# Bojian-Wei/Non-IID-Distributed-Learning-with-Optimal-Mixture-Weights

Hardware: AMD Instinct MI355X
Metric: client-rounds/sec (whole node) (higher is better)
Workload: dtype f32; 1 GPU; config 2: fedavg, 100 clients x 512 rows, RFF D=2048, C=10, E=2, B=32, 10000 test rows, round=1880, parallel clients; algo=fedavg, clients_total=100, clients_per_gpu=100, rows_per_client=512, D=2048, C=10, epochs=2, batch=32, test_rows=10000, parallelism=clients1

## Files before the change

non-iid-distributed-learning-with-optimal-mixture-weights_amd/csrc/local_train_host.cpp:

```cpp
#include <mutex>
#include <unordered_map>

#include "local_train_wide.h"
#include "split_common.h"

namespace fs {

static_assert(SP_ERR_BYTES == PR_ERR_BYTES && SP_ERR_BYTES == PP_ERR_BYTES && SP_ERR_BYTES == WD_ERR_BYTES,
              "one error block for every form");

static int device_cus() {
  static int cus = 0;
  if (cus == 0) {
    int dev = 0;
    if (hipGetDevice(&dev) != hipSuccess) return 0;
    if (hipDeviceGetAttribute(&cus, hipDeviceAttributeMultiprocessorCount, dev) != hipSuccess) cus = 0;
  }
  return cus;
}

static unsigned exchange_generation(const void* ws, bool long_launch) {
  static std::mutex gm;
  static std::unordered_map<const void*, unsigned> gens;
  std::lock_guard<std::mutex> lk(gm);
  auto it = gens.find(ws);
  const unsigned prev = it == gens.end() ? 0u : it->second;
  const unsigned gen = (long_launch || prev >= 4095u) ? 0u : prev + 1u;
  gens[ws] = gen;
  return gen;
}

static unsigned spin_bound(unsigned form_limit) {
  const fs_tuning t = tuning();
  if (t.inject_timeout) return 0u;
  return t.spin_limit ? t.spin_limit : form_limit;
}

constexpr int SPLIT_PD_WIDE = 16, SPLIT_PD_NARROW = 0;
static int split_poll_delay(int G, bool chained) {
  const int t = tuning().split_poll_delay;
  if (t < 0) return 0;
  if (t > 0) return t;
  if (chained) return 0;
  return G >= 8 ? SPLIT_PD_WIDE : SPLIT_PD_NARROW;
}


static size_t split_dyn_lds(int RT, int NT, int G, int teams) {
  const int tiles = (NT + G - 1) / G;
  return sizeof(float) * (size_t)teams * (size_t)(RT * 16) * (size_t)(tiles * 64 + 8);
}

static size_t split_static_lds(int RT, int NW, int teams) {
  const int NR = RT * 16;
  return (size_t)teams * ((size_t)NW * NR * 16 * 4 + 2 * (size_t)NR * 16 * 4 + 2 * NR * 4 + NW * 3 * 4 + 8) + 64 +
         4 * teams;
}

static bool split_fits(int C, int B, int NT, int G, int teams) {
  if (!(G == 2 || G == 4 || G == 8 || G == 16)) return false;
  if (C > 16 || B > 32 || NT < G) return false;
  const int RT = lt_rt(B);
  const int nw = SP_WAVES / teams;
  const int tiles = (NT + G - 1) / G;
  if ((tiles + nw - 1) / nw > SP_TPW) return false;
  if (G >= 8 && RT * 16 * C + 2 > 512) return false;
  return split_dyn_lds(RT, NT, G, teams) + split_static_lds(RT, nw, teams) <= 160 * 1024;
}

static size_t pair_dyn_lds(int RT) { return sizeof(float) * 2 * (size_t)(RT * 16) * (size_t)(PR_TILES * 64 + 8); }

static size_t pair_static_lds(int RT) {
  const int NR = RT * 16;
  return (size_t)PR_WAVES * NR * 16 * 4 + (size_t)NR * 16 * 4 + 2 * NR * 4 + 2 * PR_WAVES * 2 * 4 +
         PR_WAVES * 4 + 8 + 64;
}

struct Form {
  int flag;
  int kernel;
  int lanes;
  int slots;
  bool chains;
  bool poll_delay;
  unsigned spin_limit;
  size_t fuse_lds;
  bool (*fits)(int C, int B, int NT, int G);
  int (*sz)(int RT);
  size_t (*lds)(int RT, int NT, int G);
  int (*launch)(const LTParams& P, int G, const SplitWS& X, int grid, size_t lds, hipStream_t st);
  const char* unfit;
};

static int split_sz(int RT) { return RT * 16 * 16 + 4; }
constexpr size_t SPLIT_FUSE_LDS = sizeof(float) * SP_WAVES * 16 * 17;

static const Form SPLIT = {
    0, FS_LT_SPLIT, 1, 2, true, true, SP_SPIN_LIMIT, SPLIT_FUSE_LDS,
    [](int C, int B, int NT, int G) { return split_fits(C, B, NT, G, 1); }, split_sz,
    [](int RT, int NT, int G) { return split_dyn_lds(RT, NT, G, 1); }, launch_split_instance,
    "fs_local_train: slice too wide for one workgroup"};

static const Form TEAMS = {
    FS_G_TEAMS, FS_LT_TEAMS, 2, 4, false, true, SP_SPIN_LIMIT, SPLIT_FUSE_LDS,
    [](int C, int B, int NT, int G) { return (G == 4 || G == 8) && split_fits(C, B, NT, G, 2); }, split_sz,
    [](int RT, int NT, int G) { return split_dyn_lds(RT, NT, G, 2); }, launch_teams_instance,
    "fs_local_train: slice too wide for one workgroup"};

static const Form PAIR = {
    FS_G_PAIR, FS_LT_PAIR, 2, 5, false, false, PR_SPIN_LIMIT, 0,
    [](int C, int B, int NT, int G) {
      if (!(G == 2 || G == 4 || G == 8 || G == 16)) return false;
      if (C > 14 || B > 32 || NT != PR_TILES * G) return false;
      const int RT = lt_rt(B);
      return pair_dyn_lds(RT) + pair_static_lds(RT) <= 160 * 1024;
    },
    [](int RT) { return RT * 16 * 16 + 4 >= PR_THREADS ? RT * 16 * 16 + 4 : PR_THREADS; },
    [](int RT, int, int) { return pair_dyn_lds(RT); }, launch_pair_instance,
    "fs_local_train: the pair form needs C <= 14, B <= 32 and ld == 512 G"};

static const Form PIPE = {
    FS_G_PIPE, FS_LT_PIPE, 1, 2, true, false, SP_SPIN_LIMIT, 0,
    [](int C, int B, int NT, int G) {
      if (!(G == 2 || G == 4 || G == 8 || G == 16)) return false;
      return C >= 1 && C <= 16 && B > 16 && B <= 32 && NT == PP_NTS * G;
    },
    [](int) { return PP_SZ; },
    [](int, int, int) { return sizeof(float) * (size_t)PP_NR * PP_RS; }, launch_pipe_instance,
    "fs_local_train: the pipe form needs ld = 1024 G (G = 2, 4, 8 or 16), 16 < B <= 32 and C <= 16"};

static const Form& form_of(int G) {
  return (G & FS_G_PIPE) ? PIPE : (G & FS_G_PAIR) ? PAIR : (G & FS_G_TEAMS) ? TEAMS : SPLIT;
}

static int form_groups(const Form& f, int N, int G, int chained, int cus) {
  return chained ? 1 : std::max(1, std::min((N + f.lanes - 1) / f.lanes, cus / G));
}

static int64_t form_xbuf_bytes(const Form& f, int ngroups, int G, int RT) {
  return (int64_t)ngroups * f.slots * G * f.sz(RT) * 8;
}

static int64_t form_ws_bytes(const Form& f, int N, int G, int B, int chained, int cus) {
  return form_xbuf_bytes(f, form_groups(f, N, G, chained, cus), G, lt_rt(B)) + SP_ERR_BYTES;
}

int split_idle_cus(int N, int C, int B, int64_t ld, int G, int chained) {
  if (G & FS_G_WIDE) return 0;
  const Form& f = form_of(G);
  const int g = G & (FS_G_PAIR - 1);
  const int cus = device_cus();
  if (chained || cus <= 0 || !f.fits(C, B, (int)(ld >> 6), g)) return 0;
  return std::max(0, cus - form_groups(f, N, g, 0, cus) * g);
}


static int form_admits(const Form& f, const LTParams& P, int G, int NT) {
  if (&f == &TEAMS && (P.chained || !(G == 4 || G == 8)))
    return fail(FS_EUNSUPPORTED, "fs_local_train: the team form runs parallel clients at G = 4 or 8");
  if (&f == &PAIR && P.chained) return fail(FS_EINVAL, "fs_local_train: the pair form needs parallel clients");
  if (&f == &SPLIT || &f == &TEAMS) {
    if (!(G == 2 || G == 4 || G == 8 || G == 16)) return fail(FS_EINVAL, "fs_local_train: G must be 1, 2, 4, 8 or 16");
    if (P.C > 16 || P.B > 32) return fail(FS_EUNSUPPORTED, "fs_local_train: split clients need C <= 16, B <= 32");
    if (NT < G) return fail(FS_EUNSUPPORTED, "fs_local_train: fewer feature tiles than workgroups per client");
  }
  if (!f.fits(P.C, P.B, NT, G)) return fail(FS_EUNSUPPORTED, f.unfit);
  return FS_OK;
}

static int exchange_setup(const Form& f, const LTParams& P, int G, void* ws, int64_t ws_bytes, hipStream_t st,
                          SplitWS& X, int& grid, size_t& lds) {
  const int RT = lt_rt(P.B);
  const int NT = (int)(P.ld >> 6);
  if (int rc = form_admits(f, P, G, NT)) return rc;
  const int cus = device_cus();
  if (cus <= 0) return fail(FS_EHIP, "fs_local_train: no device");
  if (G > cus) return fail(FS_EUNSUPPORTED, "fs_local_train: G exceeds the CU count");
  const int ng = form_groups(f, P.N, G, P.chained, cus);
  const int64_t xbytes = form_xbuf_bytes(f, ng, G, RT);
  if (!ws || ws_bytes < xbytes + SP_ERR_BYTES) return fail(FS_EINVAL, "fs_local_train: workspace too small");
  char* base = reinterpret_cast<char*>(ws);
  X.xbuf = reinterpret_cast<unsigned long long*>(base);
  X.err = reinterpret_cast<unsigned*>(base + ws_bytes - SP_ERR_BYTES);
  X.SZ = f.sz(RT);
  X.ngroups = ng;
  X.spin_limit = spin_bound(f.spin_limit);
  X.poll_delay = f.poll_delay ? split_poll_delay(G, P.chained != 0) : 0;
  X.stamps = nullptr;
#ifdef FS_STAMPS
  X.stamps = reinterpret_cast<unsigned long long*>(base + xbytes);
#endif
  const int64_t seq_clients = P.chained ? P.N : (P.N + ng * f.lanes - 1) / (ng * f.lanes);
  const bool long_launch = P.max_client_steps <= 0 || P.max_client_steps * seq_clients >= (1 << 20) - 1;
  const unsigned gen = exchange_generation(ws, long_launch);
  X.tag_base = gen << 20;
  if (gen <= 1) {
    hipError_t e = hipMemsetAsync(base, 0, (size_t)xbytes, st);
// ... 153 lines not shown
```

non-iid-distributed-learning-with-optimal-mixture-weights_amd/csrc/local_train_split.hip:

```cpp
#include <type_traits>

#include "common.h"
#include "eval_rows.h"
#include "lanes.h"
#include "split_common.h"

namespace fs {

#ifndef SP_E1
#define SP_E1 6
#endif
#ifndef SP_E2
#define SP_E2 0
#endif
#ifndef SP_E3
#define SP_E3 0
#endif
constexpr int SP_EARLY = SP_E1 + SP_E2 + SP_E3;
#ifndef SP_BWD_FENCE
#define SP_BWD_FENCE 1
#endif
#ifndef SP_BWD_NUM
#define SP_BWD_NUM 1
#endif
#ifndef SP_BWD_DEN
#define SP_BWD_DEN 1
#endif
#ifndef SP_BWD_PF
#define SP_BWD_PF 1
#endif
#ifndef SP_EG2
#define SP_EG2 4
#endif
#ifndef SP_BWD_TAIL
#define SP_BWD_TAIL 8
#endif
#ifndef SP_BWD_TAILPER
#define SP_BWD_TAILPER 8
#endif
#ifndef SP_MB_RSP
#define SP_MB_RSP 4
#endif
#ifndef SP_MB_BWD_PF
#define SP_MB_BWD_PF 1
#endif
#ifndef SP_MB_PRE
#define SP_MB_PRE 1
#endif

#ifdef FS_STAMPS
#define SP_STAMP(k)                                                                       \
  {                                                                                       \
    __builtin_amdgcn_sched_barrier(0);                                                    \
    unsigned long long t_;                                                                \
    asm volatile("s_memtime %0\n\ts_waitcnt lgkmcnt(0)" : "=s"(t_)::"memory");           \
    __builtin_amdgcn_sched_barrier(0);                                                    \
    if (k > 0) stamp_acc[k > 0 ? k - 1 : 0] += t_ - stamp_prev;                           \
    stamp_prev = t_;                                                                      \
  }
#else
#define SP_STAMP(k)
#endif

template <int CBSZ, int ABID, int BLGP>
__device__ __forceinline__ floatx4 mfma4x4(float a, float b, floatx4 c) {
  return __builtin_amdgcn_mfma_f32_4x4x1f32(a, b, c, CBSZ, ABID, BLGP);
}
template <int Q, int RT, int CB>
__device__ __forceinline__ void mb_fwd_q(floatx4 (&acc)[RT][CB], const float4 (&xt)[RT][4], const float4 (&wt)[CB]) {
#pragma unroll
  for (int e = 0; e < 4; ++e)
#pragma unroll
    for (int rt = 0; rt < RT; ++rt)
#pragma unroll
      for (int cb = 0; cb < CB; ++cb) acc[rt][cb] = mfma4x4<2, Q, 0>(comp(wt[cb], e), comp(xt[rt][Q], e), acc[rt][cb]);
}
template <int CB>
__device__ __forceinline__ void mb_bwd_row(floatx4 (&ga)[CB], float a, float g) {
  ga[0] = mfma4x4<0, 0, 4>(a, g, ga[0]);
  if constexpr (CB > 1) ga[1] = mfma4x4<0, 0, 5>(a, g, ga[1]);
  if constexpr (CB > 2) ga[2] = mfma4x4<0, 0, 6>(a, g, ga[2]);
  if constexpr (CB > 3) ga[3] = mfma4x4<0, 0, 7>(a, g, ga[3]);
}
__device__ __forceinline__ void mb_swap32(float& a, float& b) {
  const auto r = __builtin_amdgcn_permlane32_swap(__float_as_uint(a), __float_as_uint(b), false, false);
  a = __uint_as_float(r[0]);
  b = __uint_as_float(r[1]);
}
__device__ __forceinline__ void mb_swap16(float& a, float& b) {
  const auto r = __builtin_amdgcn_permlane16_swap(__float_as_uint(a), __float_as_uint(b), false, false);
  a = __uint_as_float(r[0]);
  b = __uint_as_float(r[1]);
}
__device__ __forceinline__ float mb_kgroup_sum(floatx4 a) {
  float r0 = a[0], r1 = a[1], r2 = a[2], r3 = a[3];
  mb_swap32(r0, r1);
  mb_swap32(r2, r3);
  float s01 = r0 + r1, s23 = r2 + r3;
  mb_swap16(s01, s23);
  return s01 + s23;
}
__device__ __forceinline__ int mb_perm(int lg) { return ((lg & 1) << 1) | (lg >> 1); }
template <int CB>
__device__ __forceinline__ int zp_off_mb(int r, int c) {
  return ((r >> 4) * CB + (c >> 2)) * 64 + (c & 3) * 16 + ((r & 15) ^ ((c >> 2) << 2));
}

template <int RT, int G, bool PROX, int EARLY, int TEAMS, int WAVES = SP_WAVES, int TPWK = SP_TPW, int MBK = 0>
__global__ __launch_bounds__(WAVES * 64, 1) void local_train_split_kernel(LTParams P, SplitWS X) {
  static_assert(TEAMS == 1 || TEAMS == 2, "teams");
  static_assert(WAVES == SP_WAVES || (WAVES == 4 && TEAMS == 1), "waves");
  static_assert(MBK >= 0 && MBK <= 4 && (MBK == 0 || TEAMS == 1), "mb");
  constexpr bool MB = MBK > 0;
  constexpr int NQ = MB ? MBK : 4;
  constexpr int NCS = !MB || MBK > 2 ? 16 : 4 * MBK;
  constexpr int NW = WAVES / TEAMS;
  constexpr int NTH = NW * 64;
  constexpr int NC = 16;
  constexpr int NR = RT * 16;
  constexpr int NZ = NR * NC;
  constexpr int NZS = NR * NCS;
  constexpr int TPW = TPWK;
  constexpr int XT = NTH;
  constexpr int M = ((G >= 8 ? 512 : NZ + 2) + XT - 1) / XT;
  constexpr int HC = G;
  __shared__ __attribute__((aligned(16))) float zpart_t[TEAMS][NW][NR * NC];
  __shared__ float gbuf_t[TEAMS][NR][NC];
  __shared__ float zsum_t[TEAMS][NR][NC];
  __shared__ int lab_t[TEAMS][2][NR];
  __shared__ float wred_t[TEAMS][NW][2];
  __shared__ float wce_t[TEAMS][NW];
  __shared__ float nrm_t[TEAMS][2];
  __shared__ unsigned tbar[TEAMS];
  extern __shared__ __attribute__((aligned(16))) float xs_dyn[];

  const int team = TEAMS > 1 ? __builtin_amdgcn_readfirstlane((int)threadIdx.x / NTH) : 0;
  const int tid = (int)threadIdx.x - team * NTH, lane = tid & 63, l16 = lane & 15, lg = lane >> 4;
  const int w = __builtin_amdgcn_readfirstlane(tid >> 6);
  const int mq = (lane >> 2) & 3, mi = lane & 3;
  auto& zpart = zpart_t[team];
  auto& gbuf = gbuf_t[team];
  auto& zsum = zsum_t[team];
  auto& lab = lab_t[team];
  auto& wred = wred_t[team];
  auto& wce = wce_t[team];
  auto& nrm = nrm_t[team];
  const int64_t ld = P.ld;
  const int NT = (int)(ld >> 6);
  const int C = P.C, B = P.B, E = P.E;
  const int NV = NR * C + 2;
  static_assert(NZS % 64 == 0, "the softmax loop must stay wave-uniform");

  const int nb = gridDim.x - P.fuse_E;
  if ((int)blockIdx.x >= nb) {
    if constexpr (WAVES == SP_WAVES)
      eval_persistent<SP_WAVES>(P.fuse_phi, P.ld, P.fuse_y, P.fuse_n, P.W_start, P.C, (int)blockIdx.x - nb, P.fuse_E,
                         xs_dyn, P.fuse_part);
    return;
  }
  int lin;
  if (P.chained) {
    if (blockIdx.x % 8) return;
    lin = blockIdx.x / 8;
  } else {
    lin = blockIdx.x;
    if (nb % 8 == 0) lin = (blockIdx.x % 8) * (nb / 8) + blockIdx.x / 8;
  }
  const int ngp = X.ngroups;
  const int grpp = lin / G, g = lin % G;
  if (grpp >= ngp) return;
  const int ng = ngp * TEAMS, grp = grpp * TEAMS + team;
  const int T = P.chained ? P.N : (P.N + ng - 1) / ng;
  const int t0 = tile_lo(g, G, NT), t1 = tile_lo(g + 1, G, NT);
  const int NTS = t1 - t0;
  constexpr int RSP = MB ? SP_MB_RSP : 8;
  const int RS = NTS * 64 + RSP;
  const int xs_off = TEAMS > 1 ? team * (NR * RS) : 0;
#define xs_lds (xs_dyn + xs_off)
  const float* start = P.W_start;
  unsigned long long* xb = X.xbuf + (int64_t)grp * 2 * G * X.SZ;
  unsigned tb_target = 0;
  bool tb_dead = false;
  if (TEAMS > 1 && tid == 0) tbar[team] = 0u;
  auto team_sync = [&]() {
    if constexpr (TEAMS == 1) {
      lds_barrier();
    } else {
      tb_target += NW;
      asm volatile("s_waitcnt lgkmcnt(0)" ::: "memory");
      if (lane == 0) __hip_atomic_fetch_add(&tbar[team], 1u, __ATOMIC_RELAXED, __HIP_MEMORY_SCOPE_WORKGROUP);
      for (unsigned sp = 0; !tb_dead &&
                            __hip_atomic_load(&tbar[team], __ATOMIC_RELAXED, __HIP_MEMORY_SCOPE_WORKGROUP) < tb_target;) {
        if (++sp > 64u * SP_SPIN_LIMIT) {
          if (lane == 0) __hip_atomic_store(X.err, 1u, __ATOMIC_RELAXED, __HIP_MEMORY_SCOPE_AGENT);
          tb_dead = true;
        }
        __builtin_amdgcn_s_sleep(1);
      }
      asm volatile("" ::: "memory");
    }
  };
  const float4 zero4 = make_float4(0.f, 0.f, 0.f, 0.f);

  float4 wr[TPW][NQ];
  const float* anc = P.W_start;
  auto wbase = [&]() {
    int64_t b = MB ? (int64_t)mi * ld + 64 * t0 + 16 * mq + 4 * lg : (int64_t)l16 * ld + 64 * t0 + 4 * lg;
    asm volatile("" : "+v"(b));
    return b;
  };
  auto woff = [&](int Tl, int q) -> int64_t { return MB ? 4 * q * ld + 64 * Tl : 64 * Tl + 16 * q; };
  auto wok = [&](int Tl, int q) { return Tl < NTS && (MB ? 4 * q + mi < C : l16 < C); };
  auto load_start = [&]() {
    const int64_t base = wbase();
    float s = 0.f;
#pragma unroll
    for (int i = 0; i < TPW; ++i) {
      const int Tl = w + NW * i;
#pragma unroll
      for (int q = 0; q < NQ; ++q) {
        wr[i][q] = wok(Tl, q) ? ld4(start + base + woff(Tl, q)) : zero4;
        s = sq4_acc(s, wr[i][q].x, wr[i][q].y, wr[i][q].z, wr[i][q].w);
      }
    }
    return wave_sum_dpp(s, lane);
  };
  auto store_w = [&](float* Wj) {
    const int64_t base = wbase();
#pragma unroll
    for (int i = 0; i < TPW; ++i) {
      const int Tl = w + NW * i;
#pragma unroll
      for (int q = 0; q < NQ; ++q)
        if (wok(Tl, q)) st4(Wj + base + woff(Tl, q), wr[i][q]);
    }
  };
  const float nw0 = load_start();
  if (lane == 0) { wred[w][0] = 0.f; wred[w][1] = nw0; }

  float4 xf[TPW][RT][4];
  int pn[RT], lb[RT];
  SpCur lc;
  bool lc_ok = sp_seek(lc, P, grp, ng, T, 0);
  auto fetch_raw = [&](int* raw, int64_t& base) {
    const int e_ = lc.st / lc.nbat, s_ = lc.st - e_ * lc.nbat;
    const int b0_ = s_ * B, bc_ = min(B, lc.n - b0_);
    const int32_t* pp_ = P.perms + (int64_t)E * lc.row0 + (int64_t)e_ * lc.n + b0_;
    base = lc.row0;
#pragma unroll
    for (int rt = 0; rt < RT; ++rt) {
      const int r_ = rt * 16 + l16;
      raw[rt] = pp_[r_ < bc_ ? r_ : 0];
    }
  };
  auto fetch_rows = [&]() {
    int raw[RT];
    int64_t base;
    fetch_raw(raw, base);
#pragma unroll
    for (int rt = 0; rt < RT; ++rt) pn[rt] = (int)(base + raw[rt]);
  };
#define SP_XLOAD()                                                                   \
  {                                                                                  \
    _Pragma("unroll") for (int rt = 0; rt < RT; ++rt) {                              \
      const int64_t r_ = pn[rt];                                                     \
      if (w == 0 && lg == 0) lb[rt] = P.labels[r_];                                  \
      const float* src_ = P.phi + r_ * ld + 64 * t0 + 4 * lg;                        \
      _Pragma("unroll") for (int i = 0; i < TPW; ++i)                                \
        if (w + NW * i < NTS)                                                        \
          _Pragma("unroll") for (int q = 0; q < 4; ++q)                              \
            xf[i][rt][q] = ld4(src_ + 64 * (w + NW * i) + 16 * q);                   \
    }                                                                                \
  }
  if (lc_ok) {
    fetch_rows();
    SP_XLOAD();
    lc_ok = sp_advance(lc, P, grp, ng, T);
    if (lc_ok) fetch_rows();
  }
  if constexpr (NCS < NC)
    for (int i = tid; i < NR * NC; i += NTH) gbuf[i / NC][i % NC] = 0.f;
  __syncthreads();

  auto flush_empty = [&](int ka, int kb) {
    for (int k = ka; k < kb; ++k) {
      const int j = sp_client(P, grp, ng, k);
      if (j < 0) continue;
      float* Wj = P.W_out + (int64_t)j * C * ld;
      if (P.chained) {
        store_w(Wj);
      } else {
        const int64_t base = wbase();
#pragma unroll
        for (int i = 0; i < TPW; ++i) {
          const int Tl = w + NW * i;
#pragma unroll
          for (int q = 0; q < NQ; ++q)
            if (wok(Tl, q)) {
              const int64_t off = base + woff(Tl, q);
              st4(Wj + off, ld4(start + off));
            }
        }
      }
      if (g == 0 && tid == 0) P.loss[j] = 0.0;
    }
  };

  SpCur cc;
  bool cc_ok = sp_seek(cc, P, grp, ng, T, 0);
  flush_empty(0, cc_ok ? cc.k : T);
  unsigned gs = 0;
  bool dead = false;
  double lsum = 0.0;
#ifdef FS_STAMPS
  unsigned long long stamp_acc[10] = {0, 0, 0, 0, 0, 0, 0, 0, 0, 0}, stamp_prev = 0;
#endif
  floatx4 acc[RT];
  floatx4 accm[RT][MB ? MBK : 1];
  auto fwd_tile = [&](int i) {
    if (w + NW * i < NTS) {
      if constexpr (MB) {
        mb_fwd_q<0>(accm, xf[i], wr[i]);
        mb_fwd_q<1>(accm, xf[i], wr[i]);
        mb_fwd_q<2>(accm, xf[i], wr[i]);
        mb_fwd_q<3>(accm, xf[i], wr[i]);
      } else {
#pragma unroll
        for (int q = 0; q < 4; ++q) {
          float4 xa[RT];
#pragma unroll
          for (int rt = 0; rt < RT; ++rt) xa[rt] = xf[i][rt][q];
#pragma unroll
          for (int e4 = 0; e4 < 4; ++e4)
#pragma unroll
            for (int rt = 0; rt < RT; ++rt) acc[rt] = mfma4(comp(xa[rt], e4), comp(wr[i][q], e4), acc[rt]);
        }
      }
    }
  };
  auto fwd_tile0 = [&]() {
#pragma unroll
    for (int rt = 0; rt < RT; ++rt) {
      acc[rt] = floatx4{0.f, 0.f, 0.f, 0.f};
#pragma unroll
      for (int cb = 0; cb < (MB ? MBK : 1); ++cb) accm[rt][cb] = floatx4{0.f, 0.f, 0.f, 0.f};
    }
    fwd_tile(0);
  };
  bool pre = false;
  for (; cc_ok; ++gs) {
    const int st = cc.st, n = cc.n, nbat = cc.nbat;
    if (st == 0) {
      if (!P.chained && gs > 0) {
        (void)load_start();
        if (lane == 0) { wred[w][0] = 0.f; wred[w][1] = nw0; }
      } else if (lane == 0) {
        wred[w][0] = 0.f;
      }
      if (PROX) anc = (P.chained && cc.j > 0) ? P.W_out + (int64_t)(cc.j - 1) * C * ld : start;
      lsum = 0.0;
    }
    {
      SP_STAMP(0)
      const int e = st / nbat, s = st - e * nbat;
      const int b0 = s * B, bc = min(B, n - b0);
      const int par = gs & 1;
      const unsigned tag32 = X.tag_base + gs + 1u;
      if (w == 0 && lg == 0)
#pragma unroll
        for (int rt = 0; rt < RT; ++rt) lab[par][rt * 16 + l16] = lb[rt];
      const bool ilv = lc_ok;
      int lbn[RT], pnr[RT];
      int64_t pnb = 0;
#pragma unroll
      for (int rt = 0; rt < RT; ++rt) { lbn[rt] = lb[rt]; pnr[rt] = 0; }
      bool lcn_ok = false;
#ifndef SP_NARROW_TOP
#define SP_NARROW_TOP 0
#endif
      constexpr bool TOP_FETCH = TPW > 1 || SP_NARROW_TOP;
      auto fetch_next = [&]() {
        if (ilv) {
          if (w == 0 && lg == 0)
#pragma unroll
            for (int rt = 0; rt < RT; ++rt) lbn[rt] = P.labels[pn[rt]];
          lcn_ok = sp_advance(lc, P, grp, ng, T);
          if (lcn_ok) fetch_raw(pnr, pnb);
        }
      };
      if constexpr (TOP_FETCH) fetch_next();

#define SP_IMG_WRITE()                                                               \
  {                                                                                  \
    _Pragma("unroll") for (int i = 0; i < TPW; ++i)                                  \
      if (w + NW * i < NTS)                                                          \
        _Pragma("unroll") for (int rt = 0; rt < RT; ++rt)                            \
          _Pragma("unroll") for (int q = 0; q < 4; ++q)                              \
            st4(xs_lds + (MB ? (rt * 16 + l16) * RS + 64 * (w + NW * i) + 16 * lg + 4 * q \
                             : img_off(rt * 16 + l16, RS, w + NW * i, 4 * q + lg)),   \
                xf[i][rt][q]);                                                       \
  }

      if (!pre) fwd_tile0();
#pragma unroll
      for (int i = 1; i < TPW; ++i) fwd_tile(i);
      if constexpr (MB) {
#pragma unroll
        for (int rt = 0; rt < RT; ++rt)
#pragma unroll
          for (int cb = 0; cb < MBK; ++cb)
            zpart[w][((rt * MBK + cb) * 4 + mb_perm(lg)) * 16 + (l16 ^ (cb << 2))] = mb_kgroup_sum(accm[rt][cb]);
      } else {
#pragma unroll
        for (int rt = 0; rt < RT; ++rt)
          st4(&zpart[w][rt * 256 + lg * 64 + l16 * 4], make_float4(acc[rt][0], acc[rt][1], acc[rt][2], acc[rt][3]));
      }
      SP_STAMP(1)
      team_sync();
      SP_STAMP(2)

      {
        unsigned long long* slot = xb + ((int64_t)par * G) * X.SZ;
        const unsigned long long tag = (unsigned long long)tag32 << 32;
        float own[M], sum[M];
        unsigned long long pl[M][HC];
#pragma unroll
        for (int m = 0; m < M; ++m) {
          const int idx = tid + XT * m;
          float v = 0.f;
          if (idx < NV - 2) {
            const int r = idx / C, c = idx - r * C;
            const int zo = MB ? zp_off_mb<MB ? MBK : 1>(r, c) : zp_off(r, c);
#pragma unroll
            for (int i = 0; i < NW; ++i) v += zpart[i][zo];
          } else if (idx < NV) {
#pragma unroll
            for (int i = 0; i < NW; ++i) v += wred[i][idx - (NV - 2)];
          }
          own[m] = v;
          sum[m] = 0.f;
          if (idx < NV)
            __hip_atomic_store(slot + (int64_t)g * X.SZ + idx, tag | __float_as_uint(v), __ATOMIC_RELAXED,
                               __HIP_MEMORY_SCOPE_AGENT);
        }
        SP_STAMP(3)
        if (X.spin_limit == 0 && gs == 0 && lane == 0)
          __hip_atomic_store(X.err, 1u, __ATOMIC_RELAXED, __HIP_MEMORY_SCOPE_AGENT);
        unsigned spins = 0;
#pragma unroll
        for (int h0 = 0; h0 < G; h0 += HC) {
          auto poll = [&]() {
#pragma unroll
            for (int m = 0; m < M; ++m) {
              const int idx = tid + XT * m;
#pragma unroll
              for (int h = 0; h < HC; ++h)
                pl[m][h] = __hip_atomic_load(slot + (int64_t)(h0 + h) * X.SZ + (idx < NV ? idx : 0),
                                             __ATOMIC_RELAXED, __HIP_MEMORY_SCOPE_AGENT);
            }
          };
          if (h0 == 0)
            for (int d_ = 0; d_ < X.poll_delay; ++d_) __builtin_amdgcn_s_sleep(1);
          poll();
          if (h0 == 0) SP_IMG_WRITE();
          for (;;) {
            bool ok = true;
#pragma unroll
            for (int m = 0; m < M; ++m)
#pragma unroll
              for (int h = 0; h < HC; ++h)
                ok &= (h0 + h == g) | (tid + XT * m >= NV) | ((unsigned)(pl[m][h] >> 32) == tag32);
            if (__all(ok)) break;
            if (dead || ++spins > X.spin_limit) {
              if (lane == 0) __hip_atomic_store(X.err, 1u, __ATOMIC_RELAXED, __HIP_MEMORY_SCOPE_AGENT);
              dead = true;
              break;
            }
            __builtin_amdgcn_s_sleep(1);
            poll();
          }
#pragma unroll
          for (int m = 0; m < M; ++m)
#pragma unroll
            for (int h = 0; h < HC; ++h)
              sum[m] += (h0 + h == g) ? own[m] : __uint_as_float((unsigned)pl[m][h]);
        }
#pragma unroll
        for (int m = 0; m < M; ++m) {
          const int idx = tid + XT * m;
          if (idx < NV) {
            if (idx < NV - 2) {
              const int r = idx / C, c = idx - r * C;
              zsum[r][c] = sum[m];
            } else {
              nrm[idx - (NV - 2)] = sum[m];
            }
          }
        }
        SP_STAMP(4)
      }
      constexpr int NLD = TPW * 4 * RT;
      constexpr int NE = EARLY < NLD ? EARLY : NLD;
      auto issue_row = [&](int f) {
        const int i = f / (4 * RT), kk = f % (4 * RT);
        xf[i][kk >> 2][kk & 3] =
            ld4(P.phi + (int64_t)pn[kk >> 2] * ld + 64 * t0 + 4 * lg + 64 * (w + NW * i) + 16 * (kk & 3));
      };
      constexpr int E1 = TPW == 1 ? NE : SP_E1;
      constexpr int NE1 = E1 < NE ? E1 : NE, NE2 = E1 + SP_E2 < NE ? E1 + SP_E2 : NE;
      float4 avall[PROX && NE > 0 ? TPW : 1][NQ];
      if constexpr (PROX && NE > 0) {
        if constexpr (MB) {
          const float* ap = anc + 64 * t0 + 16 * mq + 4 * lg;
#pragma unroll
          for (int i = 0; i < TPW; ++i)
#pragma unroll
            for (int q = 0; q < NQ; ++q) avall[i][q] = ld4(ap + (int64_t)min(4 * q + mi, C - 1) * ld + 64 * (w + NW * i));
        } else {
          const float* ap = anc + (int64_t)min(l16, C - 1) * ld + 64 * t0 + 4 * lg;
#pragma unroll
          for (int i = 0; i < TPW; ++i)
#pragma unroll
            for (int q = 0; q < 4; ++q) avall[i][q] = ld4(ap + 64 * (w + NW * i) + 16 * q);
        }
      }
      if constexpr (NE > 0)
#pragma unroll
        for (int f = 0; f < NE1; ++f) issue_row(f);
      SP_STAMP(5)
      team_sync();
      if constexpr (NE > 0)
#pragma unroll
        for (int f = NE1; f < NE2; ++f) issue_row(f);
      SP_STAMP(6)
      const float invb = 1.0f / (float)bc;
      float cep = 0.f;
      for (int idx = tid; idx < NZS; idx += NTH) {
        const int r = idx / NCS, c = idx - r * NCS;
        const bool valid = r < bc && c < C;
        const float z = valid ? zsum[r][c] : 0.f;
        float m = valid ? z : -INFINITY;
#pragma unroll
        for (int off = NCS / 2; off > 0; off >>= 1) m = fmaxf(m, xor_get(m, off, lane));
        const float ex = valid ? __expf(z - m) : 0.f;
        float se = ex;
#pragma unroll
        for (int off = NCS / 2; off > 0; off >>= 1) se += xor_get(se, off, lane);
        float gv = 0.f;
        if (valid) {
          const bool isy = c == lab[par][r];
          gv = (isy ? -invb : 0.f) + ex * __builtin_amdgcn_rcpf(se) * invb;
          if (isy) cep -= z - m - __logf(se);
        }
        gbuf[r][c] = gv;
      }
      cep = wave_sum_dpp(cep, lane);
      if (lane == 0) wce[w] = cep;
      team_sync();
      if constexpr (NE > 0)
#pragma unroll
        for (int f = NE2; f < NE; ++f) issue_row(f);
      SP_STAMP(7)
      const float pn2 = nrm[0], wn2 = nrm[1];
      if (g == 0 && tid == 0 && e == E - 1) {
        float ce = 0.f;
        for (int i = 0; i < NW; ++i) ce += wce[i];
        float loss = ce / (float)bc;
        if (P.prox) loss = loss + P.mu * sqrtf(pn2);
        if (P.reg) loss = loss + P.lam * sqrtf(wn2);
        lsum += (double)loss * (double)bc;
      }

      float gB[MB ? 1 : 4 * RT];
      if constexpr (!MB)
#pragma unroll
        for (int kk = 0; kk < 4 * RT; ++kk) gB[kk] = gbuf[4 * kk + lg][l16];
      const float sp = (P.prox && pn2 > 0.f) ? P.mu / sqrtf(pn2) : 0.f;
      const float sr = (P.reg && wn2 > 0.f) ? P.lam / sqrtf(wn2) : 0.f;
      const float lr = P.lr;
      const int rblk = 4 * (l16 & 3) + (l16 >> 2);
      float npn = 0.f, nwn = 0.f;
      auto bwd = [&](auto LD, auto FULL, auto EA) {
        constexpr int EAN = decltype(EA)::value;
      if constexpr (MB) {
        constexpr int RS_FULL = NW * TPW * 64 + RSP;
        const int RSx = decltype(FULL)::value ? RS_FULL : RS;
        float4 av[TPW][NQ];
        if constexpr (PROX && EAN > 0) {
#pragma unroll
          for (int i = 0; i < TPW; ++i)
#pragma unroll
            for (int q = 0; q < NQ; ++q) av[i][q] = avall[i][q];
        } else if constexpr (PROX) {
#pragma unroll
          for (int i = 0; i < TPW; ++i)
#pragma unroll
            for (int q = 0; q < NQ; ++q) {
              const int Tl = w + NW * i;
              av[i][q] = wok(Tl, q) ? ld4(anc + wbase() + woff(Tl, q)) : zero4;
            }
        }
        floatx4 gm[TPW][NQ];
#pragma unroll
        for (int i = 0; i < TPW; ++i)
#pragma unroll
          for (int q = 0; q < NQ; ++q) gm[i][q] = floatx4{0.f, 0.f, 0.f, 0.f};
        if constexpr (decltype(FULL)::value && SP_MB_BWD_PF > 0) {
          float xa[2][4][TPW], gq[2][4];
          auto rd = [&](int kk, int b) {
#pragma unroll
            for (int rr = 0; rr < 4; ++rr) {
#ifdef SP_MB_DIAG_NOGREAD
              gq[b][rr] = gbuf[0][4 * lg + mi] + (float)(kk + rr);
#else
              gq[b][rr] = gbuf[4 * kk + rr][4 * lg + mi];
#endif
#pragma unroll
              for (int i = 0; i < TPW; ++i)
#ifdef SP_MB_DIAG_NOXREAD
                xa[b][rr][i] = (float)(kk * 4 + rr + i) * gq[b][rr];
#else
                xa[b][rr][i] = xs_lds[(4 * kk + rr) * RSx + 64 * (w + NW * i) + lane];
#endif
            }
          };
          rd(0, 0);
#pragma unroll
          for (int kk = 0; kk < 4 * RT; ++kk) {
            if (kk + 1 < 4 * RT) rd(kk + 1, (kk + 1) & 1);
            __builtin_amdgcn_sched_barrier(0);
#pragma unroll
            for (int rr = 0; rr < 4; ++rr)
#pragma unroll
              for (int i = 0; i < TPW; ++i) mb_bwd_row<MBK>(gm[i], xa[kk & 1][rr][i], gq[kk & 1][rr]);
            if constexpr (decltype(LD)::value) {
#pragma unroll
              for (int i = 0; i < TPW; ++i) {
                const int f = kk * TPW + i + EAN;
                if (f < NLD) issue_row(f);
              }
            }
            __builtin_amdgcn_sched_barrier(0);
          }
        } else
#pragma unroll
        for (int kk = 0; kk < 4 * RT; ++kk) {
#pragma unroll
          for (int rr = 0; rr < 4; ++rr) {
            const int r = 4 * kk + rr;
            const float gv = gbuf[r][4 * lg + mi];
#pragma unroll
            for (int i = 0; i < TPW; ++i) {
              const int Tl = w + NW * i;
              if (decltype(FULL)::value || Tl < NTS)
                mb_bwd_row<MBK>(gm[i], xs_lds[r * RSx + 64 * Tl + lane], gv);
            }
          }
          if constexpr (decltype(LD)::value) {
#pragma unroll
            for (int i = 0; i < TPW; ++i) {
              const int f = kk * TPW + i + EAN;
              if (f < NLD && (decltype(FULL)::value || w + NW * (f / (4 * RT)) < NTS)) issue_row(f);
            }
          }
        }
#pragma unroll
        for (int i = 0; i < TPW; ++i) {
          const int Tl = w + NW * i;
#pragma unroll
          for (int q = 0; q < NQ; ++q)
            if ((decltype(FULL)::value || Tl < NTS) && 4 * q + mi < C) {
              float o[4];
#pragma unroll
              for (int e4 = 0; e4 < 4; ++e4) {
                const float wc = comp(wr[i][q], e4);
                const float ac = PROX ? comp(av[i][q], e4) : 0.f;
                o[e4] = sgd_w(wc, gm[i][q][e4], lr, PROX, ac, sp, P.reg, sr);
                if (PROX) {
                  const float dp = o[e4] - ac;
                  npn = sq_acc(npn, dp);
                  nwn = sq_acc(nwn, o[e4]);
                }
              }
              wr[i][q] = make_float4(o[0], o[1], o[2], o[3]);
            }
        }
      } else {
#pragma unroll
      for (int i = 0; i < TPW; ++i) {
        const int Tl = w + NW * i;
        if (decltype(FULL)::value || Tl < NTS) {
          float4 av[4];
          if constexpr (PROX && EAN > 0) {
#pragma unroll
            for (int q = 0; q < 4; ++q) av[q] = avall[i][q];
          } else if (PROX && l16 < C) {
            const float* ap = anc + wbase() + 64 * Tl;
#pragma unroll
            for (int q = 0; q < 4; ++q) av[q] = ld4(ap + 16 * q);
          }
          floatx4 ga[4];
#pragma unroll
          for (int e4 = 0; e4 < 4; ++e4) ga[e4] = floatx4{0.f, 0.f, 0.f, 0.f};
          constexpr int RS_FULL = NW * TPW * 64 + 8;
          const int RSx = decltype(FULL)::value ? RS_FULL : RS;
          const float* ib0 = xs_lds + lg * RSx + 64 * Tl + 4 * (rblk ^ lg);
          const float* ib1 = xs_lds + lg * RSx + 64 * Tl + 4 * (rblk ^ (lg + 4));
          float4 xpre[TPW == 1 ? 4 * RT : 1];
          if constexpr (TPW == 1) {
#pragma unroll
            for (int kk = 0; kk < 4 * RT; ++kk) xpre[kk] = ld4(((kk & 1) ? ib1 : ib0) + 4 * kk * RSx);
            __builtin_amdgcn_sched_barrier(0);
          }
          constexpr bool FENCED =
              SP_BWD_FENCE && RT == 2 && G == 2 && !PROX && TEAMS == 1 && TPW > 1 && EAN > 0 && EAN < NLD;
          constexpr bool PF = FENCED && SP_BWD_PF;
          float4 xn = zero4;
          if constexpr (PF) xn = ld4(ib0);
#pragma unroll
          for (int kk = 0; kk < 4 * RT; ++kk) {
            float4 x;
            if constexpr (PF) {
              x = xn;
              if (kk + 1 < 4 * RT) xn = ld4((((kk + 1) & 1) ? ib1 : ib0) + 4 * (kk + 1) * RSx);
              __builtin_amdgcn_sched_barrier(0);
            } else {
              x = TPW == 1 ? xpre[kk] : ld4(((kk & 1) ? ib1 : ib0) + 4 * kk * RSx);
            }
#pragma unroll
            for (int e4 = 0; e4 < 4; ++e4) ga[e4] = mfma4(comp(x, e4), gB[kk], ga[e4]);
            if constexpr (decltype(LD)::value) {
              if constexpr (EAN == 0) {
                xf[i][kk >> 2][kk & 3] = ld4(P.phi + (int64_t)pn[kk >> 2] * ld + 64 * t0 + 4 * lg + 64 * Tl + 16 * (kk & 3));
              } else if constexpr (FENCED) {
                constexpr int NIT = TPW * 4 * RT;
                const int it = i * 4 * RT + kk;
#pragma unroll
                for (int f = EAN; f < NLD; ++f) {
                  const int head = ((f - EAN + 1) * SP_BWD_DEN + SP_BWD_NUM - 1) / SP_BWD_NUM - 1;
                  const int itf = f < NLD - SP_BWD_TAIL ? (head < NIT ? head : NIT - 1) : NIT - 1 - (NLD - 1 - f) / SP_BWD_TAILPER;
                  if (itf == it) issue_row(f);
                }
                __builtin_amdgcn_sched_barrier(0);
              } else {
                if (i * 4 * RT + kk + EAN < NLD) issue_row(i * 4 * RT + kk + EAN);
              }
            }
          }
          if (l16 < C) {
#pragma unroll
            for (int q = 0; q < 4; ++q) {
              float o[4];
#pragma unroll
              for (int e4 = 0; e4 < 4; ++e4) {
                const float wc = comp(wr[i][q], e4);
                const float ac = PROX ? comp(av[q], e4) : 0.f;
                o[e4] = sgd_w(wc, ga[e4][q], lr, PROX, ac, sp, P.reg, sr);
                if (PROX) {
                  const float dp = o[e4] - ac;
                  npn = sq_acc(npn, dp);
                  nwn = sq_acc(nwn, o[e4]);
                }
              }
              wr[i][q] = make_float4(o[0], o[1], o[2], o[3]);
            }
          }
        }
      }
      }
      };
      using E0 = std::integral_constant<int, 0>;
      if constexpr (NE > 0) {
        bwd(std::true_type{}, std::true_type{}, std::integral_constant<int, NE>{});
      } else if (ilv) {
        if (NTS == NW * TPW)
          bwd(std::true_type{}, std::true_type{}, E0{});
        else
          bwd(std::true_type{}, std::false_type{}, E0{});
      } else {
        bwd(std::false_type{}, std::false_type{}, E0{});
      }
      if constexpr (!TOP_FETCH) fetch_next();
      if (ilv) {
#pragma unroll
        for (int rt = 0; rt < RT; ++rt) {
          lb[rt] = lbn[rt];
          if (lcn_ok) pn[rt] = (int)(pnb + pnr[rt]);
        }
        lc_ok = lcn_ok;
      }
      if (!PROX && P.reg) {
#pragma unroll
        for (int i = 0; i < TPW; ++i)
#pragma unroll
          for (int q = 0; q < NQ; ++q)
#pragma unroll
            for (int e4 = 0; e4 < 4; ++e4) nwn = sq_acc(nwn, comp(wr[i][q], e4));
      }
      if (PROX || P.reg) {
        npn = PROX ? wave_sum_dpp(npn, lane) : 0.f;
        nwn = wave_sum_dpp(nwn, lane);
        if (lane == 0) { wred[w][0] = npn; wred[w][1] = nwn; }
      }
      constexpr bool PRE_OK = !MB || (SP_MB_PRE && ((MBK <= 2 && G <= 8) || (MBK == 3 && G == 2 && !PROX)));
      pre = TEAMS == 1 && TPW > 1 && PRE_OK && st + 1 < cc.steps;
      if (pre) fwd_tile0();
      SP_STAMP(8)
    }
    if (st == cc.steps - 1) {
      store_w(P.W_out + (int64_t)cc.j * C * ld);
      if (g == 0 && tid == 0) P.loss[cc.j] = lsum / (double)n;
    }
    const int kprev = cc.k;
    cc_ok = sp_advance(cc, P, grp, ng, T);
    flush_empty(kprev + 1, cc_ok ? cc.k : T);
  }
#undef SP_XLOAD
#undef SP_IMG_WRITE
#undef xs_lds
#ifdef FS_STAMPS
  if (threadIdx.x == 0 && X.stamps) {
    for (int k = 0; k < 8; ++k) X.stamps[blockIdx.x * 16 + k] = stamp_acc[k];
    X.stamps[blockIdx.x * 16 + 15] = (unsigned long long)gs;
  }
#endif
}

#ifndef FS_SPLIT_KERNEL_ONLY
template <int RT, int G, bool PROX, int EARLY, int TEAMS, int WAVES = SP_WAVES, int TPWK = SP_TPW, int MBK = 0>
static void launch_split_k(const LTParams& P, const SplitWS& X, int grid, size_t lds, hipStream_t st) {
  if (lds > 64 * 1024)
    (void)hipFuncSetAttribute(
        reinterpret_cast<const void*>(&local_train_split_kernel<RT, G, PROX, EARLY, TEAMS, WAVES, TPWK, MBK>),
        hipFuncAttributeMaxDynamicSharedMemorySize, (int)lds);
  hipLaunchKernelGGL((local_train_split_kernel<RT, G, PROX, EARLY, TEAMS, WAVES, TPWK, MBK>), dim3(grid),
                     dim3(WAVES * 64), lds, st, P, X);
}

static int split_mbk(const LTParams& P, int G, int teams) {
  const int t = tuning().split_mb;
  if (t < 0 || teams != 1 || lt_rt(P.B) != 2) return 0;
  const int cb = (P.C + 3) / 4;
  if (t == 0 && cb > 2 && !(cb == 3 && G >= 16)) return 0;
  return cb;
}

template <int RT, int G, bool PROX, int EARLY, int TEAMS, int WAVES = SP_WAVES, int TPWK = SP_TPW>
static void launch_split_s(const LTParams& P, const SplitWS& X, int grid, size_t lds, hipStream_t st) {
  if constexpr (RT == 2 && TEAMS == 1) {
    switch (split_mbk(P, G, TEAMS)) {
      case 1: set_last_lt_kernel(FS_LT_MB); launch_split_k<RT, G, PROX, EARLY, TEAMS, WAVES, TPWK, 1>(P, X, grid, lds, st); return;
      case 2: set_last_lt_kernel(FS_LT_MB); launch_split_k<RT, G, PROX, EARLY, TEAMS, WAVES, TPWK, 2>(P, X, grid, lds, st); return;
      case 3: set_last_lt_kernel(FS_LT_MB); launch_split_k<RT, G, PROX, EARLY, TEAMS, WAVES, TPWK, 3>(P, X, grid, lds, st); return;
      case 4: set_last_lt_kernel(FS_LT_MB); launch_split_k<RT, G, PROX, EARLY, TEAMS, WAVES, TPWK, 4>(P, X, grid, lds, st); return;
      default: break;
    }
  }
  launch_split_k<RT, G, PROX, EARLY, TEAMS, WAVES, TPWK, 0>(P, X, grid, lds, st);
}

constexpr int SPLIT_NARROW_EARLY = 8;
template <int RT, int G>
static bool launch_split_narrow(const LTParams& P, const SplitWS& X, int grid, size_t lds, hipStream_t st) {
  if constexpr (RT != 2 || G < 4) {
    return false;
  } else {
    const int64_t NT = P.ld >> 6;
    if (!P.chained || P.fuse_E > 0 || tuning().split_early < 0) return false;
    if (NT == 4 * G) {
      const size_t l4 = std::max(lds, (size_t)96 * 1024);
      if (P.prox) launch_split_s<RT, G, true, SPLIT_NARROW_EARLY, 1, 4, 1>(P, X, grid, l4, st);
      else launch_split_s<RT, G, false, SPLIT_NARROW_EARLY, 1, 4, 1>(P, X, grid, l4, st);
      return true;
    }
    if (NT == 8 * G) {
      if (P.prox) launch_split_s<RT, G, true, SPLIT_NARROW_EARLY, 1, SP_WAVES, 1>(P, X, grid, lds, st);
      else launch_split_s<RT, G, false, SPLIT_NARROW_EARLY, 1, SP_WAVES, 1>(P, X, grid, lds, st);
      return true;
    }
    return false;
  }
}

template <int RT, int G>
static void launch_split_teams(const LTParams& P, const SplitWS& X, int grid, size_t lds, hipStream_t st) {
  constexpr int EARLY_G = SP_EARLY;
  const bool full = (P.ld >> 6) == (int64_t)G * (SP_WAVES / 2) * SP_TPW;
  if (P.prox) launch_split_s<RT, G, true, 0, 2>(P, X, grid, lds, st);
  else if (full && EARLY_G > 0 && tuning().split_early >= 0) launch_split_s<RT, G, false, EARLY_G, 2>(P, X, grid, lds, st);
  else launch_split_s<RT, G, false, 0, 2>(P, X, grid, lds, st);
}

bool dbuf_covers(int C, int B, int64_t ld, int G, int chained, int prox, int* waves_out);
int launch_local_train_dbuf(const LTParams& P, int G, const SplitWS& X, int grid, size_t lds, hipStream_t st);
static bool dbuf_by_shape(const LTParams& P, int G) {
  if (tuning().split_dbuf <= 0 || tuning().split_early < 0) return false;
  return dbuf_covers(P.C, P.B, P.ld, G, P.chained, P.prox, nullptr);
}

template <int RT, int G>
static void launch_split_g(const LTParams& P, const SplitWS& X, int grid, size_t lds, hipStream_t st) {
  if (RT == 2 && dbuf_by_shape(P, G) && launch_local_train_dbuf(P, G, X, grid, lds, st) == FS_OK) {
    set_last_lt_kernel(FS_LT_DBUF);
    return;
  }
  constexpr int EARLY_G = (G == 2 && SP_EARLY > SP_EG2) ? SP_EG2 : SP_EARLY;
#ifndef SP_EP
#define SP_EP 2
#endif
  constexpr int EARLY_PROX = SP_EARLY < SP_EP ? SP_EARLY : SP_EP;
  const bool full = (P.ld >> 6) == (int64_t)G * SP_WAVES * SP_TPW;
  const bool early = full && EARLY_G > 0 && tuning().split_early >= 0;
  if (launch_split_narrow<RT, G>(P, X, grid, lds, st)) return;
  if (P.prox && early) launch_split_s<RT, G, true, EARLY_PROX, 1>(P, X, grid, lds, st);
  else if (P.prox) launch_split_s<RT, G, true, 0, 1>(P, X, grid, lds, st);
  else if (early) launch_split_s<RT, G, false, EARLY_G, 1>(P, X, grid, lds, st);
  else launch_split_s<RT, G, false, 0, 1>(P, X, grid, lds, st);
}

int launch_split_instance(const LTParams& P, int G, const SplitWS& X, int grid, size_t lds, hipStream_t st) {
  const int RT = lt_rt(P.B);
#define FS_SPLIT_CASE(rt, g) \
  if (RT == rt && G == g) { launch_split_g<rt, g>(P, X, grid, lds, st); return FS_OK; }
  FS_SPLIT_CASE(2, 2) FS_SPLIT_CASE(2, 4) FS_SPLIT_CASE(2, 8) FS_SPLIT_CASE(2, 16)
  FS_SPLIT_CASE(1, 2) FS_SPLIT_CASE(1, 4) FS_SPLIT_CASE(1, 8) FS_SPLIT_CASE(1, 16)
#undef FS_SPLIT_CASE
  return fail(FS_EUNSUPPORTED, "fs_local_train: no split kernel for this shape");
}

int launch_teams_instance(const LTParams& P, int G, const SplitWS& X, int grid, size_t lds, hipStream_t st) {
  const int RT = lt_rt(P.B);
  if (RT == 2 && G == 4) { launch_split_teams<2, 4>(P, X, grid, lds, st); return FS_OK; }
  if (RT == 2 && G == 8) { launch_split_teams<2, 8>(P, X, grid, lds, st); return FS_OK; }
  if (RT == 1 && G == 4) { launch_split_teams<1, 4>(P, X, grid, lds, st); return FS_OK; }
  if (RT == 1 && G == 8) { launch_split_teams<1, 8>(P, X, grid, lds, st); return FS_OK; }
  return fail(FS_EUNSUPPORTED, "fs_local_train: no team kernel for this shape");
}
#endif

}
```

Measured before the change: 376,400 client-rounds/s.

## Trim split-kernel exchange slots, skip norm slots, DPP row max, incremental epoch/step

Several micro-optimizations land in the split local-train kernel. The exchange slot count M is now sized from the class count (up to 15, with a C16 instantiation for larger C), and the two norm slots are dropped when neither prox nor reg is active. The softmax row max uses a hand-written DPP sequence, and epoch/step indices are tracked incrementally instead of by division. The cross-entropy accumulation runs only in the last epoch, and the reciprocal batch size is precomputed. The poll delay for G=4 also rises to the wide value, and G=2 gets a nonzero delay. The inline asm and the extra template instantiations add risk.

```diff
diff --git a/non-iid-distributed-learning-with-optimal-mixture-weights_amd/csrc/local_train_host.cpp b/non-iid-distributed-learning-with-optimal-mixture-weights_amd/csrc/local_train_host.cpp
--- a/non-iid-distributed-learning-with-optimal-mixture-weights_amd/csrc/local_train_host.cpp
+++ b/non-iid-distributed-learning-with-optimal-mixture-weights_amd/csrc/local_train_host.cpp
@@ -36,13 +36,13 @@
   return t.spin_limit ? t.spin_limit : form_limit;
 }
 
-constexpr int SPLIT_PD_WIDE = 16, SPLIT_PD_NARROW = 0;
+constexpr int SPLIT_PD_WIDE = 16, SPLIT_PD_G2 = 4;
 static int split_poll_delay(int G, bool chained) {
   const int t = tuning().split_poll_delay;
   if (t < 0) return 0;
   if (t > 0) return t;
   if (chained) return 0;
-  return G >= 8 ? SPLIT_PD_WIDE : SPLIT_PD_NARROW;
+  return G >= 4 ? SPLIT_PD_WIDE : SPLIT_PD_G2;
 }
 
 
diff --git a/non-iid-distributed-learning-with-optimal-mixture-weights_amd/csrc/local_train_split.hip b/non-iid-distributed-learning-with-optimal-mixture-weights_amd/csrc/local_train_split.hip
--- a/non-iid-distributed-learning-with-optimal-mixture-weights_amd/csrc/local_train_split.hip
+++ b/non-iid-distributed-learning-with-optimal-mixture-weights_amd/csrc/local_train_split.hip
@@ -106,8 +106,34 @@
   return ((r >> 4) * CB + (c >> 2)) * 64 + (c & 3) * 16 + ((r & 15) ^ ((c >> 2) << 2));
 }
 
-template <int RT, int G, bool PROX, int EARLY, int TEAMS, int WAVES = SP_WAVES, int TPWK = SP_TPW, int MBK = 0>
+constexpr int SP_C1 = 15;
+constexpr int SP_MBK_C16 = 8;
+template <int RT, int G, int XT, int MBK, bool C16>
+constexpr int split_slots() {
+  constexpr int cmax = (MBK > 0 && MBK < 4) ? 4 * MBK : (C16 ? 16 : SP_C1);
+  constexpr int nv = RT * 16 * cmax + 2;
+  return ((G >= 8 && nv > 512 ? 512 : nv) + XT - 1) / XT;
+}
+__device__ __forceinline__ float sp_row16_max(float x) {
+  float r;
+  asm volatile(
+      "s_nop 1\n\t"
+      "v_max_f32_dpp %0, %1, %1 row_ror:8 row_mask:0xf bank_mask:0xf\n\t"
+      "s_nop 1\n\t"
+      "v_max_f32_dpp %0, %0, %0 row_ror:4 row_mask:0xf bank_mask:0xf\n\t"
+      "s_nop 1\n\t"
+      "v_max_f32_dpp %0, %0, %0 quad_perm:[2,3,0,1] row_mask:0xf bank_mask:0xf\n\t"
+      "s_nop 1\n\t"
+      "v_max_f32_dpp %0, %0, %0 quad_perm:[1,0,3,2] row_mask:0xf bank_mask:0xf"
+      : "=&v"(r)
+      : "v"(x));
+  return r;
+}
+
+template <int RT, int G, bool PROX, int EARLY, int TEAMS, int WAVES = SP_WAVES, int TPWK = SP_TPW, int MBKC = 0>
 __global__ __launch_bounds__(WAVES * 64, 1) void local_train_split_kernel(LTParams P, SplitWS X) {
+  constexpr int MBK = MBKC & 7;
+  constexpr bool C16 = (MBKC & SP_MBK_C16) != 0;
   static_assert(TEAMS == 1 || TEAMS == 2, "teams");
   static_assert(WAVES == SP_WAVES || (WAVES == 4 && TEAMS == 1), "waves");
   static_assert(MBK >= 0 && MBK <= 4 && (MBK == 0 || TEAMS == 1), "mb");
@@ -122,7 +148,7 @@
   constexpr int NZS = NR * NCS;
   constexpr int TPW = TPWK;
   constexpr int XT = NTH;
-  constexpr int M = ((G >= 8 ? 512 : NZ + 2) + XT - 1) / XT;
+  constexpr int M = split_slots<RT, G, XT, MBK, C16>();
   constexpr int HC = G;
   __shared__ __attribute__((aligned(16))) float zpart_t[TEAMS][NW][NR * NC];
   __shared__ float gbuf_t[TEAMS][NR][NC];
@@ -148,7 +174,8 @@
   const int64_t ld = P.ld;
   const int NT = (int)(ld >> 6);
   const int C = P.C, B = P.B, E = P.E;
-  const int NV = NR * C + 2;
+  const bool NRM = P.prox || P.reg;
+  const int NL = NR * C, NV = NL + (NRM ? 2 : 0);
   static_assert(NZS % 64 == 0, "the softmax loop must stay wave-uniform");
 
   const int nb = gridDim.x - P.fuse_E;
@@ -242,8 +269,14 @@
   int pn[RT], lb[RT];
   SpCur lc;
   bool lc_ok = sp_seek(lc, P, grp, ng, T, 0);
+  struct SpES { int e, s; };
+  auto es_next = [](SpES& p, const SpCur& c) {
+    if (c.st == 0) { p.e = 0; p.s = 0; }
+    else if (++p.s == c.nbat) { p.s = 0; ++p.e; }
+  };
+  SpES lces = {0, 0};
   auto fetch_raw = [&](int* raw, int64_t& base) {
-    const int e_ = lc.st / lc.nbat, s_ = lc.st - e_ * lc.nbat;
+    const int e_ = lces.e, s_ = lces.s;
     const int b0_ = s_ * B, bc_ = min(B, lc.n - b0_);
     const int32_t* pp_ = P.perms + (int64_t)E * lc.row0 + (int64_t)e_ * lc.n + b0_;
     base = lc.row0;
@@ -276,7 +309,7 @@
     fetch_rows();
     SP_XLOAD();
     lc_ok = sp_advance(lc, P, grp, ng, T);
-    if (lc_ok) fetch_rows();
+    if (lc_ok) { es_next(lces, lc); fetch_rows(); }
   }
   if constexpr (NCS < NC)
     for (int i = tid; i < NR * NC; i += NTH) gbuf[i / NC][i % NC] = 0.f;
@@ -308,6 +341,9 @@
 
   SpCur cc;
   bool cc_ok = sp_seek(cc, P, grp, ng, T, 0);
+  SpES cces = {0, 0};
+  const float inv_full = 1.0f / (float)B;
+  float inv_tail = 0.f;
   flush_empty(0, cc_ok ? cc.k : T);
   unsigned gs = 0;
   bool dead = false;
@@ -359,11 +395,13 @@
       }
       if (PROX) anc = (P.chained && cc.j > 0) ? P.W_out + (int64_t)(cc.j - 1) * C * ld : start;
       lsum = 0.0;
+      inv_tail = 1.0f / (float)(n - (nbat - 1) * B);
     }
     {
       SP_STAMP(0)
-      const int e = st / nbat, s = st - e * nbat;
+      const int e = cces.e, s = cces.s;
       const int b0 = s * B, bc = min(B, n - b0);
+      const bool last_e = e == E - 1;
       const int par = gs & 1;
       const unsigned tag32 = X.tag_base + gs + 1u;
       if (w == 0 && lg == 0)
@@ -385,7 +423,7 @@
 #pragma unroll
             for (int rt = 0; rt < RT; ++rt) lbn[rt] = P.labels[pn[rt]];
           lcn_ok = sp_advance(lc, P, grp, ng, T);
-          if (lcn_ok) fetch_raw(pnr, pnb);
+          if (lcn_ok) { es_next(lces, lc); fetch_raw(pnr, pnb); }
         }
       };
       if constexpr (TOP_FETCH) fetch_next();
@@ -428,14 +466,17 @@
         for (int m = 0; m < M; ++m) {
           const int idx = tid + XT * m;
           float v = 0.f;
-          if (idx < NV - 2) {
+          if (idx < NL) {
             const int r = idx / C, c = idx - r * C;
             const int zo = MB ? zp_off_mb<MB ? MBK : 1>(r, c) : zp_off(r, c);
 #pragma unroll
             for (int i = 0; i < NW; ++i) v += zpart[i][zo];
           } else if (idx < NV) {
-#pragma unroll
-            for (int i = 0; i < NW; ++i) v += wred[i][idx - (NV - 2)];
+            float t[NW];
+#pragma unroll
+            for (int i = 0; i < NW; ++i) t[i] = wred[i][idx - NL];
+#pragma unroll
+            for (int i = 0; i < NW; ++i) v += t[i];
           }
           own[m] = v;
           sum[m] = 0.f;
@@ -489,11 +530,11 @@
         for (int m = 0; m < M; ++m) {
           const int idx = tid + XT * m;
           if (idx < NV) {
-            if (idx < NV - 2) {
+            if (idx < NL) {
               const int r = idx / C, c = idx - r * C;
               zsum[r][c] = sum[m];
             } else {
-              nrm[idx - (NV - 2)] = sum[m];
+              nrm[idx - NL] = sum[m];
             }
           }
         }
@@ -533,15 +574,19 @@
 #pragma unroll
         for (int f = NE1; f < NE2; ++f) issue_row(f);
       SP_STAMP(6)
-      const float invb = 1.0f / (float)bc;
+      const float invb = s == nbat - 1 ? inv_tail : inv_full;
       float cep = 0.f;
       for (int idx = tid; idx < NZS; idx += NTH) {
         const int r = idx / NCS, c = idx - r * NCS;
         const bool valid = r < bc && c < C;
         const float z = valid ? zsum[r][c] : 0.f;
         float m = valid ? z : -INFINITY;
-#pragma unroll
-        for (int off = NCS / 2; off > 0; off >>= 1) m = fmaxf(m, xor_get(m, off, lane));
+        if constexpr (NCS == 16) {
+          m = sp_row16_max(m);
+        } else {
+#pragma unroll
+          for (int off = NCS / 2; off > 0; off >>= 1) m = fmaxf(m, xor_get(m, off, lane));
+        }
         const float ex = valid ? __expf(z - m) : 0.f;
         float se = ex;
 #pragma unroll
@@ -550,19 +595,21 @@
         if (valid) {
           const bool isy = c == lab[par][r];
           gv = (isy ? -invb : 0.f) + ex * __builtin_amdgcn_rcpf(se) * invb;
-          if (isy) cep -= z - m - __logf(se);
         }
         gbuf[r][c] = gv;
-      }
-      cep = wave_sum_dpp(cep, lane);
-      if (lane == 0) wce[w] = cep;
+        if (last_e && valid && c == lab[par][r]) cep -= z - m - __logf(se);
+      }
+      if (last_e) {
+        cep = wave_sum_dpp(cep, lane);
+        if (lane == 0) wce[w] = cep;
+      }
       team_sync();
       if constexpr (NE > 0)
 #pragma unroll
         for (int f = NE2; f < NE; ++f) issue_row(f);
       SP_STAMP(7)
-      const float pn2 = nrm[0], wn2 = nrm[1];
-      if (g == 0 && tid == 0 && e == E - 1) {
+      const float pn2 = NRM ? nrm[0] : 0.f, wn2 = NRM ? nrm[1] : 0.f;
+      if (g == 0 && tid == 0 && last_e) {
         float ce = 0.f;
         for (int i = 0; i < NW; ++i) ce += wce[i];
         float loss = ce / (float)bc;
@@ -813,6 +860,7 @@
     }
     const int kprev = cc.k;
     cc_ok = sp_advance(cc, P, grp, ng, T);
+    if (cc_ok) es_next(cces, cc);
     flush_empty(kprev + 1, cc_ok ? cc.k : T);
   }
 #undef SP_XLOAD
@@ -829,6 +877,13 @@
 #ifndef FS_SPLIT_KERNEL_ONLY
 template <int RT, int G, bool PROX, int EARLY, int TEAMS, int WAVES = SP_WAVES, int TPWK = SP_TPW, int MBK = 0>
 static void launch_split_k(const LTParams& P, const SplitWS& X, int grid, size_t lds, hipStream_t st) {
+  constexpr int XT = WAVES / TEAMS * 64;
+  if constexpr (MBK < SP_MBK_C16 && split_slots<RT, G, XT, MBK, true>() != split_slots<RT, G, XT, MBK, false>()) {
+    if (P.C > SP_C1) {
+      launch_split_k<RT, G, PROX, EARLY, TEAMS, WAVES, TPWK, MBK | SP_MBK_C16>(P, X, grid, lds, st);
+      return;
+    }
+  }
   if (lds > 64 * 1024)
     (void)hipFuncSetAttribute(
         reinterpret_cast<const void*>(&local_train_split_kernel<RT, G, PROX, EARLY, TEAMS, WAVES, TPWK, MBK>),
```

Result: faster. 387,100 client-rounds/s (median of 6 runs) (+2.8%).
